# NVlabs/InstantSplat

Measured on AMD Instinct MI355X. Metric: train_iters_per_sec, higher is better.
Workload: dtype f32

## Files before the change

instantsplat_amd/csrc/adam.hip:

```cpp
#include <math.h>
#include "common.h"

namespace {

__global__ __launch_bounds__(256) void k_adam(int64_t n, int row, float* __restrict__ param, const float* __restrict__ grad,
                                               float* __restrict__ exp_avg, float* __restrict__ exp_avg_sq,
                                               const float* __restrict__ per_point_lr, const float* __restrict__ grad_sumsq,
                                               float step_size, float beta1, float beta2, float eps) {
  const bool update = grad_sumsq ? (*grad_sumsq > 0.f) : true;
  const int64_t stride = (int64_t)gridDim.x * blockDim.x;
  for (int64_t i = (int64_t)blockIdx.x * blockDim.x + threadIdx.x; i < n; i += stride) {
    float m = exp_avg[i];
    if (!update && m == 0.f) continue;
    float v = exp_avg_sq[i];
    if (update) {
      const float g = grad[i];
      m = m * beta1 + g * (1.f - beta1);
      v = v * beta2 + g * g * (1.f - beta2);
      exp_avg[i] = m;
      exp_avg_sq[i] = v;
    }
    const float denom = sqrtf(v) + eps;
    const float s = per_point_lr ? step_size * per_point_lr[i / row] : step_size;
    param[i] = param[i] - s * (m / denom);
  }
}

}

namespace {

constexpr int MT_MAX = 8;
constexpr int MT_CHUNK = 2048;

struct MultiAdamArgs {
  int n;
  int first_block[MT_MAX + 1];
  long long numel[MT_MAX];
  int row[MT_MAX];
  float* param[MT_MAX];
  const float* grad[MT_MAX];
  float* m[MT_MAX];
  float* v[MT_MAX];
  const float* pplr[MT_MAX];
  float step_size[MT_MAX];
  const float* gate;
  int gidx[MT_MAX];
  int sq_out[MT_MAX];
  int vec4[MT_MAX];
  uint32_t* live;
  uint32_t seq;
  const uint32_t* commit_count;
  unsigned long long commit_capacity;
  uint32_t* commit_poison;
};

__device__ __forceinline__ int mt_find(const MultiAdamArgs& a, int b) {
  int t = 0;
#pragma unroll
  for (int k = 1; k < MT_MAX; ++k) t += (k < a.n && b >= a.first_block[k]) ? 1 : 0;
  return t;
}

__global__ __launch_bounds__(256) void k_adam_sumsq(MultiAdamArgs a, float* __restrict__ sumsq) {
  __shared__ float s_red[4];
  const int t = mt_find(a, blockIdx.x);
  const long long lo = (long long)(blockIdx.x - a.first_block[t]) * MT_CHUNK;
  const long long hi = min(a.numel[t], lo + MT_CHUNK);
  const float* g = a.grad[t];
  float acc = 0.f;
  if (a.vec4[t]) {
    for (long long j = (lo >> 2) + threadIdx.x; j < (hi >> 2); j += 256) {
      const float4 x = reinterpret_cast<const float4*>(g)[j];
      acc += (x.x * x.x + x.y * x.y) + (x.z * x.z + x.w * x.w);
    }
  } else {
    for (long long i = lo + threadIdx.x; i < hi; i += 256) { const float x = g[i]; acc += x * x; }
  }
  acc = gs_wave_sum_row3(acc);
  if ((threadIdx.x & 63) == 63) s_red[threadIdx.x >> 6] = acc;
  __syncthreads();
  if (threadIdx.x == 0) {
    const float tot = (s_red[0] + s_red[1]) + (s_red[2] + s_red[3]);
    if (!(tot == 0.f)) atomicAdd(&sumsq[a.sq_out[t]], tot);
  }
}

__global__ __launch_bounds__(256) void k_adam_multi(MultiAdamArgs a, const float* __restrict__ sumsq, float beta1, float beta2,
                                                     float eps) {
  if (a.commit_count) {
    const bool over = (unsigned long long)*a.commit_count > a.commit_capacity;
    if (over || (a.commit_poison && *a.commit_poison)) {
      if (over && a.commit_poison && blockIdx.x == 0 && threadIdx.x == 0) *a.commit_poison = 1u;
      return;
    }
  }
  const int t = mt_find(a, blockIdx.x);
  const long long lo = (long long)(blockIdx.x - a.first_block[t]) * MT_CHUNK;
  const long long hi = min(a.numel[t], lo + MT_CHUNK);
  bool update;
  if (a.gidx[t] == -2) {
    __shared__ int s_any, s_nan;
    if (threadIdx.x == 0) { s_any = 0; s_nan = 0; }
    __syncthreads();
    bool nz = false, nan = false;
    for (long long i = lo + threadIdx.x; i < hi; i += 256) { const float x = a.grad[t][i]; nz = nz || x * x > 0.f; nan = nan || x != x; }
    if (nz) s_any = 1;
    if (nan) s_nan = 1;
    __syncthreads();
    update = s_any != 0 && s_nan == 0;
  } else {
    update = (a.gidx[t] >= 0 ? a.gate[a.gidx[t]] : sumsq[t]) > 0.f;
  }
  if (a.live) {
    const bool first = blockIdx.x == (unsigned)a.first_block[t] && threadIdx.x == 0;
    if (update) {
      if (first) { a.live[2 * t] = 0u; a.live[2 * t + 1] = 0u; }
    } else {
      const uint32_t scanned = a.live[2 * t], nonzero = a.live[2 * t + 1];
      if (scanned != 0u && scanned != a.seq && nonzero == 0u) return;
      if (first) a.live[2 * t] = a.seq;
    }
  }
  bool met_nonzero = false;
  float* __restrict__ p = a.param[t];
  const float* __restrict__ g = a.grad[t];
  float* __restrict__ mm = a.m[t];
  float* __restrict__ vv = a.v[t];
  const float* __restrict__ pplr = a.pplr[t];
  const int row = a.row[t];
  const float step_size = a.step_size[t];
  auto one = [&](float& pv, float gi, float& m, float& v, long long i) {
    if (update) {
      m = m * beta1 + gi * (1.f - beta1);
      v = v * beta2 + gi * gi * (1.f - beta2);
    }
    const float denom = sqrtf(v) + eps;
    const float s = pplr ? step_size * pplr[i / row] : step_size;
    pv = pv - s * (m / denom);
  };
  if (a.vec4[t]) {
    const long long vlo = lo >> 2, vhi = hi >> 2;
    for (long long j = vlo + threadIdx.x; j < vhi; j += 256) {
      float4 m4 = reinterpret_cast<const float4*>(mm)[j];
      if (!update && m4.x == 0.f && m4.y == 0.f && m4.z == 0.f && m4.w == 0.f) continue;
      met_nonzero = true;
      float4 v4 = reinterpret_cast<const float4*>(vv)[j];
      float4 p4 = reinterpret_cast<const float4*>(p)[j];
      float4 g4 = make_float4(0.f, 0.f, 0.f, 0.f);
      if (update) g4 = reinterpret_cast<const float4*>(g)[j];
      one(p4.x, g4.x, m4.x, v4.x, 4 * j); one(p4.y, g4.y, m4.y, v4.y, 4 * j + 1);
      one(p4.z, g4.z, m4.z, v4.z, 4 * j + 2); one(p4.w, g4.w, m4.w, v4.w, 4 * j + 3);
      if (update) { reinterpret_cast<float4*>(mm)[j] = m4; reinterpret_cast<float4*>(vv)[j] = v4; }
      reinterpret_cast<float4*>(p)[j] = p4;
    }
    if (a.live && !update && met_nonzero) a.live[2 * t + 1] = 1u;
    return;
  }
  for (long long i = lo + threadIdx.x; i < hi; i += 256) {
    float m = mm[i];
    if (!update && m == 0.f) continue;
    met_nonzero = true;
    float v = vv[i], pv = p[i];
    const float gi = update ? g[i] : 0.f;
    one(pv, gi, m, v, i);
    if (update) { mm[i] = m; vv[i] = v; }
    p[i] = pv;
  }
  if (a.live && !update && met_nonzero) a.live[2 * t + 1] = 1u;
}

}

extern "C" int mi355gs_adam_multi_step(void* stream_, int ntensors, const int64_t* numel, const int32_t* row, float* const* params,
                                       const float* const* grads, float* const* exp_avg, float* const* exp_avg_sq,
                                       const float* const* per_point_lr, const float* lr, float beta1, float beta2, float eps,
                                       const int32_t* step, float* scratch, const float* gate, const int32_t* gate_index,
                                       uint32_t* live, uint32_t seq) {
  GS_RANGE();
  hipStream_t stream = (hipStream_t)stream_;
  const int debug = 0;
  if (ntensors < 0 || ntensors > MT_MAX || (gate && !gate_index)) return MI355GS_EINVAL;
  if (ntensors == 0) return MI355GS_OK;
  if (!numel || !row || !params || !grads || !exp_avg || !exp_avg_sq || !per_point_lr || !lr || !step) return MI355GS_EINVAL;
  MultiAdamArgs a;
  a.n = ntensors; a.gate = gate;
  int blocks = 0;
  bool any_ungated = false;
  bool need_sumsq = false;
  for (int t = 0; t < MT_MAX; ++t) {
    a.first_block[t] = blocks;
    if (t < ntensors) {
      if (numel[t] < 0 || row[t] <= 0 || step[t] <= 0 || (numel[t] > 0 && (!params[t] || !grads[t] || !exp_avg[t] || !exp_avg_sq[t])))
        return MI355GS_EINVAL;
      if (gate && gate_index[t] >= MT_MAX) return MI355GS_EINVAL;
      a.numel[t] = numel[t]; a.row[t] = row[t]; a.gidx[t] = (gate && gate_index[t] >= 0) ? gate_index[t] : -1; a.sq_out[t] = t;
      if (a.gidx[t] < 0) any_ungated = true;
      a.param[t] = params[t]; a.grad[t] = grads[t]; a.m[t] = exp_avg[t]; a.v[t] = exp_avg_sq[t]; a.pplr[t] = per_point_lr[t];
      const double bc1 = 1.0 - pow((double)beta1, (double)step[t]), bc2 = 1.0 - pow((double)beta2, (double)step[t]);
      a.step_size[t] = (float)((double)lr[t] * (sqrt(bc2) / bc1));
      a.vec4[t] = (numel[t] % 4 == 0 && (((uintptr_t)params[t] | (uintptr_t)grads[t] | (uintptr_t)exp_avg[t] | (uintptr_t)exp_avg_sq[t]) & 15) == 0) ? 1 : 0;
      blocks += (int)((numel[t] + MT_CHUNK - 1) / MT_CHUNK);
    } else {
      a.numel[t] = 0; a.row[t] = 1; a.param[t] = nullptr; a.grad[t] = nullptr; a.m[t] = nullptr; a.v[t] = nullptr; a.pplr[t] = nullptr;
      a.step_size[t] = 0.f; a.vec4[t] = 0; a.gidx[t] = -1; a.sq_out[t] = t;
    }
  }
  a.first_block[MT_MAX] = blocks;
  a.live = nullptr; a.seq = 0; a.commit_count = nullptr; a.commit_capacity = 0; a.commit_poison = nullptr;
  if (blocks == 0) return MI355GS_OK;
  if (!gate && g_fused.gate == scratch) {
    a.live = g_fused.adam_live; a.seq = g_fused.adam_seq;
    a.commit_count = g_fused.commit_count; a.commit_capacity = g_fused.commit_capacity; a.commit_poison = g_fused.commit_poison;
  } else if (live && seq != 0u) {
    a.live = live; a.seq = seq;
  }
  if (gate && any_ungated) {
    for (int t = 0; t < ntensors; ++t) {
      if (a.gidx[t] >= 0) continue;
      if (a.numel[t] <= MT_CHUNK) a.gidx[t] = -2; else need_sumsq = true;
    }
  } else if (any_ungated) {
    need_sumsq = true;
  }
  if (need_sumsq && !scratch) return MI355GS_EINVAL;
  if (gate) {
    if (need_sumsq) {
      MultiAdamArgs s = a;
      int k = 0, sblocks = 0;
      for (int t = 0; t < ntensors; ++t) {
        if (a.gidx[t] != -1) continue;
        s.first_block[k] = sblocks; s.numel[k] = a.numel[t]; s.grad[k] = a.grad[t]; s.vec4[k] = a.vec4[t]; s.sq_out[k] = t;
        sblocks += (int)((a.numel[t] + MT_CHUNK - 1) / MT_CHUNK);
        ++k;
      }
      for (int j = k; j <= MT_MAX; ++j) s.first_block[j] = sblocks;
      s.n = k;
      if (hipMemsetAsync(scratch, 0, MT_MAX * sizeof(float), stream) != hipSuccess) return MI355GS_ELAUNCH;
      if (sblocks > 0) {
        GS_KRANGE("adam_sumsq");
        hipLaunchKernelGGL(k_adam_sumsq, dim3(sblocks), dim3(256), 0, stream, s, scratch);
        GS_CHECK_LAUNCH("adam_sumsq");
      }
    }
  } else if (g_fused.gate == scratch) {
    a.gate = scratch;
    for (int t = 0; t < ntensors; ++t) a.gidx[t] = t;
  } else {
    if (hipMemsetAsync(scratch, 0, MT_MAX * sizeof(float), stream) != hipSuccess) return MI355GS_ELAUNCH;
    GS_KRANGE("adam_sumsq");
    hipLaunchKernelGGL(k_adam_sumsq, dim3(blocks), dim3(256), 0, stream, a, scratch);
    GS_CHECK_LAUNCH("adam_sumsq");
  }
  GS_KRANGE("adam_multi");
  hipLaunchKernelGGL(k_adam_multi, dim3(blocks), dim3(256), 0, stream, a, (const float*)scratch, beta1, beta2, eps);
  GS_CHECK_LAUNCH("adam_multi");
  return MI355GS_OK;
}

extern "C" int mi355gs_adam_step(void* stream_, int64_t n, int row, float* param, const float* grad, float* exp_avg,
                                 float* exp_avg_sq, const float* per_point_lr, const float* grad_sumsq, float lr, float beta1,
                                 float beta2, float eps, int step) {
  GS_RANGE();
  hipStream_t stream = (hipStream_t)stream_;
  const int debug = 0;
  if (n < 0 || row <= 0 || step <= 0 || (n > 0 && (!param || !grad || !exp_avg || !exp_avg_sq))) return MI355GS_EINVAL;
  if (n == 0) return MI355GS_OK;
  const double bc1 = 1.0 - pow((double)beta1, (double)step), bc2 = 1.0 - pow((double)beta2, (double)step);
  const float step_size = (float)((double)lr * (sqrt(bc2) / bc1));
  int64_t blocks = (n + 255) / 256;
  if (blocks > 2048 * 4) blocks = 2048 * 4;
  GS_KRANGE("adam");
  hipLaunchKernelGGL(k_adam, dim3((unsigned)blocks), dim3(256), 0, stream, n, row, param, grad, exp_avg, exp_avg_sq, per_point_lr,
                     grad_sumsq, step_size, beta1, beta2, eps);
  GS_CHECK_LAUNCH("adam");
  return MI355GS_OK;
}
```

instantsplat_amd/csrc/preprocess.hip:

```cpp
#include "pose_math.h"

namespace {

constexpr float SH_C0 = 0.28209479177387814f;
constexpr float SH_C1 = 0.4886025119029199f;
constexpr float SH_C2_0 = 1.0925484305920792f, SH_C2_1 = -1.0925484305920792f, SH_C2_2 = 0.31539156525252005f,
                SH_C2_3 = -1.0925484305920792f, SH_C2_4 = 0.5462742152960396f;
constexpr float SH_C3_0 = -0.5900435899266435f, SH_C3_1 = 2.890611442640554f, SH_C3_2 = -0.4570457994644658f,
                SH_C3_3 = 0.3731763325901154f, SH_C3_4 = -0.4570457994644658f, SH_C3_5 = 1.445305721320277f,
                SH_C3_6 = -0.5900435899266435f;

struct Cov2D {
  float a, b, c;
};

struct Ewa {
  float tx, ty, tz, xmul, ymul;
  float M[6];
};

__device__ __forceinline__ Ewa ewa_setup(float3 pv, const float* view, const CamParams& cp) {
  Ewa e;
  const float limx = 1.3f * cp.tanfovx, limy = 1.3f * cp.tanfovy;
  const float txtz = pv.x / pv.z, tytz = pv.y / pv.z;
  e.tx = fminf(limx, fmaxf(-limx, txtz)) * pv.z;
  e.ty = fminf(limy, fmaxf(-limy, tytz)) * pv.z;
  e.tz = pv.z;
  e.xmul = (txtz < -limx || txtz > limx) ? 0.f : 1.f;
  e.ymul = (tytz < -limy || tytz > limy) ? 0.f : 1.f;
  const float j00 = cp.focal_x / e.tz, j02 = -(cp.focal_x * e.tx) / (e.tz * e.tz);
  const float j11 = cp.focal_y / e.tz, j12 = -(cp.focal_y * e.ty) / (e.tz * e.tz);
  e.M[0] = j00 * view[0] + j02 * view[2];
  e.M[1] = j00 * view[4] + j02 * view[6];
  e.M[2] = j00 * view[8] + j02 * view[10];
  e.M[3] = j11 * view[1] + j12 * view[2];
  e.M[4] = j11 * view[5] + j12 * view[6];
  e.M[5] = j11 * view[9] + j12 * view[10];
  return e;
}

__device__ __forceinline__ Cov2D ewa_cov2d(const Ewa& e, const float* cov) {
  const float* M = e.M;
  float MS[6];
  MS[0] = M[0] * cov[0] + M[1] * cov[1] + M[2] * cov[2];
  MS[1] = M[0] * cov[1] + M[1] * cov[3] + M[2] * cov[4];
  MS[2] = M[0] * cov[2] + M[1] * cov[4] + M[2] * cov[5];
  MS[3] = M[3] * cov[0] + M[4] * cov[1] + M[5] * cov[2];
  MS[4] = M[3] * cov[1] + M[4] * cov[3] + M[5] * cov[4];
  MS[5] = M[3] * cov[2] + M[4] * cov[4] + M[5] * cov[5];
  Cov2D c;
  c.a = MS[0] * M[0] + MS[1] * M[1] + MS[2] * M[2] + 0.3f;
  c.b = MS[0] * M[3] + MS[1] * M[4] + MS[2] * M[5];
  c.c = MS[3] * M[3] + MS[4] * M[4] + MS[5] * M[5] + 0.3f;
  return c;
}

__device__ __forceinline__ void quat_to_R(float r, float x, float y, float z, float* R) {
  R[0] = 1.f - 2.f * (y * y + z * z); R[1] = 2.f * (x * y - r * z); R[2] = 2.f * (x * z + r * y);
  R[3] = 2.f * (x * y + r * z); R[4] = 1.f - 2.f * (x * x + z * z); R[5] = 2.f * (y * z - r * x);
  R[6] = 2.f * (x * z - r * y); R[7] = 2.f * (y * z + r * x); R[8] = 1.f - 2.f * (x * x + y * y);
}

template <int NB>
__device__ __forceinline__ void sh_basis(float x, float y, float z, float* b) {
  b[0] = SH_C0;
  if (NB > 1) { b[1] = -SH_C1 * y; b[2] = SH_C1 * z; b[3] = -SH_C1 * x; }
  if (NB > 4) {
    const float xx = x * x, yy = y * y, zz = z * z, xy = x * y, yz = y * z, xz = x * z;
    b[4] = SH_C2_0 * xy; b[5] = SH_C2_1 * yz; b[6] = SH_C2_2 * (2.f * zz - xx - yy);
    b[7] = SH_C2_3 * xz; b[8] = SH_C2_4 * (xx - yy);
    if (NB > 9) {
      b[9] = SH_C3_0 * y * (3.f * xx - yy); b[10] = SH_C3_1 * xy * z;
      b[11] = SH_C3_2 * y * (4.f * zz - xx - yy); b[12] = SH_C3_3 * z * (2.f * zz - 3.f * xx - 3.f * yy);
      b[13] = SH_C3_4 * x * (4.f * zz - xx - yy); b[14] = SH_C3_5 * z * (xx - yy);
      b[15] = SH_C3_6 * x * (xx - 3.f * yy);
    }
  }
}

template <int NB>
__device__ __forceinline__ float3 sh_eval(const float* sh , float x, float y, float z) {
  float b[NB];
  sh_basis<NB>(x, y, z, b);
  float3 acc = make_float3(0.f, 0.f, 0.f);
#pragma unroll
  for (int k = 0; k < NB; ++k) {
    acc.x += b[k] * sh[3 * k]; acc.y += b[k] * sh[3 * k + 1]; acc.z += b[k] * sh[3 * k + 2];
  }
  return acc;
}

template <bool POSED, int D>
__global__ __launch_bounds__(256) void k_preprocess_fwd(
    int P, int M, const float* __restrict__ means3D, const float* __restrict__ shs, const float* __restrict__ shs_rest,
    const float* __restrict__ colors_precomp, const float* __restrict__ opacities, const float* __restrict__ scales,
    const float* __restrict__ rotations, const float* __restrict__ cov3D_precomp, CamParams cp,
    int32_t* __restrict__ radii, GsRec* __restrict__ recs, float* __restrict__ cov3Ds, uint2* __restrict__ rects,
    uint8_t* __restrict__ clamped, float* __restrict__ depths, uint8_t* __restrict__ visible, GsPosed posed, GsPrologue pro) {
  const int i = blockIdx.x * blockDim.x + threadIdx.x;
  {
    const size_t gid = (size_t)i, stride = (size_t)gridDim.x * blockDim.x;
    if (pro.grad_records) {
      const float4 z = make_float4(0.f, 0.f, 0.f, 0.f);
      for (size_t k = gid; k < pro.n_vec; k += stride) pro.grad_records[k] = z;
    }
    if (pro.tile_counters)
      for (size_t k = gid; k < (size_t)pro.n_counters; k += stride) pro.tile_counters[k] = 0u;
    if (pro.g_poses && gid < (size_t)pro.n_pose) pro.g_poses[gid] = 0.f;
    if (pro.pose_scratch && gid < 32) pro.pose_scratch[gid] = 0.f;
    if (pro.adam_scratch && gid < 8) pro.adam_scratch[gid] = 0.f;
  }
  if (i >= P) return;
  radii[i] = 0;
  if (visible) visible[i] = 0;
  rects[i] = make_uint2(0u, 0u);
  const float* view = cp.view;
  const float* proj = cp.proj;
  PoseMat pm;
  if (POSED) pm = load_pose(posed.pose);
  float3 m = make_float3(means3D[3 * (size_t)i], means3D[3 * (size_t)i + 1], means3D[3 * (size_t)i + 2]);
  if (POSED) m = pose_mean(pm, m.x, m.y, m.z);
  const float3 pv = gs_tp43(view, m);
  if (pv.z <= 0.2f) return;
  const float4 ph = gs_tp44(proj, m);
  const float pw = 1.0f / (ph.w + 0.0000001f);
  const float ndcx = ph.x * pw, ndcy = ph.y * pw;

  float cov[6];
  if (cov3D_precomp) {
#pragma unroll
    for (int k = 0; k < 6; ++k) cov[k] = cov3D_precomp[6 * (size_t)i + k];
  } else {
    float4 q = *reinterpret_cast<const float4*>(rotations + 4 * (size_t)i);
    float sc[3] = {scales[3 * (size_t)i], scales[3 * (size_t)i + 1], scales[3 * (size_t)i + 2]};
    if (POSED) {
      q = pose_rot(pm, q);
#pragma unroll
      for (int k = 0; k < 3; ++k) sc[k] = pose_scale(sc[k]);
    }
    float R[9];
    quat_to_R(q.x, q.y, q.z, q.w, R);
    const float s0 = cp.scale_modifier * sc[0], s1 = cp.scale_modifier * sc[1], s2 = cp.scale_modifier * sc[2];
    float L[9];
#pragma unroll
    for (int r = 0; r < 3; ++r) { L[3 * r] = R[3 * r] * s0; L[3 * r + 1] = R[3 * r + 1] * s1; L[3 * r + 2] = R[3 * r + 2] * s2; }
    cov[0] = L[0] * L[0] + L[1] * L[1] + L[2] * L[2];
    cov[1] = L[0] * L[3] + L[1] * L[4] + L[2] * L[5];
    cov[2] = L[0] * L[6] + L[1] * L[7] + L[2] * L[8];
    cov[3] = L[3] * L[3] + L[4] * L[4] + L[5] * L[5];
    cov[4] = L[3] * L[6] + L[4] * L[7] + L[5] * L[8];
    cov[5] = L[6] * L[6] + L[7] * L[7] + L[8] * L[8];
  }
#pragma unroll
  for (int k = 0; k < 6; ++k) cov3Ds[6 * (size_t)i + k] = cov[k];

  const Ewa e = ewa_setup(pv, view, cp);
  const Cov2D c2 = ewa_cov2d(e, cov);
  const float det = c2.a * c2.c - c2.b * c2.b;
  if (det == 0.0f) return;
  const float det_inv = 1.f / det;
  const float ca = c2.c * det_inv, cb = -c2.b * det_inv, cc = c2.a * det_inv;
  const float mid = 0.5f * (c2.a + c2.c);
  const float sq = sqrtf(fmaxf(0.1f, mid * mid - det));
  const float radius = ceilf(3.f * sqrtf(fmaxf(mid + sq, mid - sq)));
  const float px = ((ndcx + 1.0f) * cp.W - 1.0f) * 0.5f, py = ((ndcy + 1.0f) * cp.H - 1.0f) * 0.5f;
  const int rminx = min(cp.gx, max(0, (int)((px - radius) / GS_TILE)));
  const int rminy = min(cp.gy, max(0, (int)((py - radius) / GS_TILE)));
  const int rmaxx = min(cp.gx, max(0, (int)((px + radius + GS_TILE - 1) / GS_TILE)));
  const int rmaxy = min(cp.gy, max(0, (int)((py + radius + GS_TILE - 1) / GS_TILE)));
  if ((rmaxx - rminx) * (rmaxy - rminy) == 0) return;

  float3 rgb;
  uint8_t clamp_bits = 0;
  if (colors_precomp) {
    rgb = make_float3(colors_precomp[3 * (size_t)i], colors_precomp[3 * (size_t)i + 1], colors_precomp[3 * (size_t)i + 2]);
  } else {
    float dx = m.x - cp.campos[0], dy = m.y - cp.campos[1], dz = m.z - cp.campos[2];
    const float inv = 1.0f / sqrtf(dx * dx + dy * dy + dz * dz);
    dx *= inv; dy *= inv; dz *= inv;
    float3 v;
    constexpr int NBF = (D + 1) * (D + 1);
    if (shs_rest == nullptr) {
      v = sh_eval<NBF>(shs + (size_t)i * M * 3, dx, dy, dz);
    } else {
      float shl[NBF * 3];
      shl[0] = shs[3 * (size_t)i]; shl[1] = shs[3 * (size_t)i + 1]; shl[2] = shs[3 * (size_t)i + 2];
      const float* rest = shs_rest + (size_t)i * (M - 1) * 3;
#pragma unroll
      for (int k = 3; k < NBF * 3; ++k) shl[k] = rest[k - 3];
      v = sh_eval<NBF>(shl, dx, dy, dz);
    }
    v.x += 0.5f; v.y += 0.5f; v.z += 0.5f;
    clamp_bits = (uint8_t)((v.x < 0.f ? 1 : 0) | (v.y < 0.f ? 2 : 0) | (v.z < 0.f ? 4 : 0));
    rgb = make_float3(fmaxf(v.x, 0.f), fmaxf(v.y, 0.f), fmaxf(v.z, 0.f));
  }

  const float opac = POSED ? pose_opacity(opacities[i]) : opacities[i];
  float hx, hy;
  const float tau = __logf(255.0f * opac);
  const float cdet = ca * cc - cb * cb;
  if (!(tau > 0.f)) { hx = hy = -1e30f; }
  else if (!(cdet > 0.f) || ca * cc > 1000.f * cdet) { hx = hy = 1e30f; }
  else {
    const float s = 2.f * tau / cdet;
    hx = sqrtf(s * cc) * 1.01f + 0.5f;
    hy = sqrtf(s * ca) * 1.01f + 0.5f;
  }

  radii[i] = (int)radius;
  if (visible) visible[i] = 1;
  clamped[i] = clamp_bits;
  int bminx = rminx, bminy = rminy, bmaxx = rmaxx, bmaxy = rmaxy;
  if (hx < 1e29f) {
    if (hx < 0.f) { bmaxx = bminx; bmaxy = bminy; }
    else {
      bminx = max(bminx, (int)floorf((px - hx) * (1.0f / GS_TILE)));
      bminy = max(bminy, (int)floorf((py - hy) * (1.0f / GS_TILE)));
      bmaxx = min(bmaxx, (int)floorf((px + hx) * (1.0f / GS_TILE)) + 1);
      bmaxy = min(bmaxy, (int)floorf((py + hy) * (1.0f / GS_TILE)) + 1);
      if (bmaxx <= bminx || bmaxy <= bminy) { bmaxx = bminx; bmaxy = bminy; }
    }
  }
  rects[i] = make_uint2((uint32_t)bminx | ((uint32_t)bminy << 16), (uint32_t)bmaxx | ((uint32_t)bmaxy << 16));
  GsRec rec;
  rec.q0 = make_float4(px, py, hx, hy);
  rec.q1 = make_float4(-0.5f * GS_LOG2E * ca, -0.5f * GS_LOG2E * cc, -GS_LOG2E * cb, opac);
  rec.q2 = make_float4(rgb.x, rgb.y, rgb.z, pv.z);
  recs[i] = rec;
  depths[i] = pv.z;
}

template <int NB>
__device__ __forceinline__ void sh_backward(const float* sh, float* gsh, float x, float y, float z, float3 gr, float* gd) {
  float b[NB];
  sh_basis<NB>(x, y, z, b);
#pragma unroll
  for (int k = 0; k < NB; ++k) { gsh[3 * k] = b[k] * gr.x; gsh[3 * k + 1] = b[k] * gr.y; gsh[3 * k + 2] = b[k] * gr.z; }
  float w[NB];
#pragma unroll
  for (int k = 0; k < NB; ++k) w[k] = sh[3 * k] * gr.x + sh[3 * k + 1] * gr.y + sh[3 * k + 2] * gr.z;
  float gx = 0.f, gy = 0.f, gz = 0.f;
  if (NB > 1) { gy += -SH_C1 * w[1]; gz += SH_C1 * w[2]; gx += -SH_C1 * w[3]; }
  if (NB > 4) {
    const float xx = x * x, yy = y * y, zz = z * z;
    gx += SH_C2_0 * y * w[4]; gy += SH_C2_0 * x * w[4];
    gy += SH_C2_1 * z * w[5]; gz += SH_C2_1 * y * w[5];
    gx += SH_C2_2 * -2.f * x * w[6]; gy += SH_C2_2 * -2.f * y * w[6]; gz += SH_C2_2 * 4.f * z * w[6];
    gx += SH_C2_3 * z * w[7]; gz += SH_C2_3 * x * w[7];
    gx += SH_C2_4 * 2.f * x * w[8]; gy += SH_C2_4 * -2.f * y * w[8];
    if (NB > 9) {
      gx += SH_C3_0 * 6.f * x * y * w[9]; gy += SH_C3_0 * (3.f * xx - 3.f * yy) * w[9];
      gx += SH_C3_1 * y * z * w[10]; gy += SH_C3_1 * x * z * w[10]; gz += SH_C3_1 * x * y * w[10];
      gx += SH_C3_2 * -2.f * x * y * w[11]; gy += SH_C3_2 * (4.f * zz - xx - 3.f * yy) * w[11]; gz += SH_C3_2 * 8.f * y * z * w[11];
      gx += SH_C3_3 * -6.f * x * z * w[12]; gy += SH_C3_3 * -6.f * y * z * w[12]; gz += SH_C3_3 * (6.f * zz - 3.f * xx - 3.f * yy) * w[12];
      gx += SH_C3_4 * (4.f * zz - 3.f * xx - yy) * w[13]; gy += SH_C3_4 * -2.f * x * y * w[13]; gz += SH_C3_4 * 8.f * x * z * w[13];
      gx += SH_C3_5 * 2.f * x * z * w[14]; gy += SH_C3_5 * -2.f * y * z * w[14]; gz += SH_C3_5 * (xx - yy) * w[14];
      gx += SH_C3_6 * (3.f * xx - 3.f * yy) * w[15]; gy += SH_C3_6 * -6.f * x * y * w[15];
    }
  }
  gd[0] = gx; gd[1] = gy; gd[2] = gz;
}

template <bool POSED, int D, bool POSE_ONLY = false>
__global__ __launch_bounds__(256) void k_preprocess_bwd(
    int P, int M, const float* __restrict__ means3D, const float* __restrict__ shs, const float* __restrict__ shs_rest,
    const float* __restrict__ scales, const float* __restrict__ rotations, int use_shs, int use_cov_precomp, CamParams cp, const int32_t* __restrict__ radii,
    const GsRec* __restrict__ recs, const float* __restrict__ cov3Ds, const uint8_t* __restrict__ clamped, const GsGrad* __restrict__ grads,
    float* __restrict__ dL_dmeans3D, float* __restrict__ dL_dmeans2D, float* __restrict__ dL_dshs, float* __restrict__ dL_dshs_rest,
    float* __restrict__ dL_dcolors, float* __restrict__ dL_dopac, float* __restrict__ dL_dscales,
    float* __restrict__ dL_drots, float* __restrict__ dL_dcov3D, float* __restrict__ sh_gate, float* __restrict__ sh_rest_gate,
    GsPosed posed, float* __restrict__ gate, int gi_xyz, int gi_rot, int gi_scaling, int gi_opacity) {
  __shared__ float s_red[POSED ? 4 : 1][16];
  const int i_raw = blockIdx.x * blockDim.x + threadIdx.x;
  if (!POSED && i_raw >= P) return;
  const bool live = i_raw < P;
  const int i = live ? i_raw : 0;
  const bool vis = live && radii[i] > 0;
  PoseMat pm;
  if (POSED) pm = load_pose(posed.pose);
  GsGrad g;
  g.g0 = make_float4(0, 0, 0, 0); g.g1 = g.g0; g.g2 = g.g0;
  if (vis) {
    const GsGrad mo = grads[i];
    const float4 pre = recs[i].q1;
    const float4 con = make_float4(pre.x * (-2.0f / GS_LOG2E), pre.z * (-1.0f / GS_LOG2E), pre.y * (-2.0f / GS_LOG2E), pre.w);
    const float m1 = mo.g0.x, m2 = mo.g0.y, m3 = mo.g0.z, m4 = mo.g0.w, m5 = mo.g1.x, m0 = mo.g1.y;
    g.g0.x = -(con.x * m1 + con.y * m2) * (0.5f * cp.W);
    g.g0.y = -(con.z * m2 + con.y * m1) * (0.5f * cp.H);
    g.g0.z = -0.5f * m3;
    g.g0.w = -m4;
    g.g1.x = -0.5f * m5;
    g.g1.y = con.w != 0.f ? m0 / con.w : 0.f;
    g.g1.z = mo.g1.z; g.g1.w = mo.g1.w; g.g2.x = mo.g2.x;
  }
  float gm[3] = {0.f, 0.f, 0.f};
  float gcov[6] = {0.f, 0.f, 0.f, 0.f, 0.f, 0.f};
  float gs[3] = {0.f, 0.f, 0.f}, gq[4] = {0.f, 0.f, 0.f, 0.f};
  const float3 gcol = make_float3(g.g1.z, g.g1.w, g.g2.x);
  constexpr int nb = (D + 1) * (D + 1);
  const bool split = shs_rest != nullptr;
  float gsh_local[nb * 3];

  if (vis) {
    const float* view = cp.view;
    const float* proj = cp.proj;
    float3 m = make_float3(means3D[3 * (size_t)i], means3D[3 * (size_t)i + 1], means3D[3 * (size_t)i + 2]);
    if (POSED) m = pose_mean(pm, m.x, m.y, m.z);
    float cov[6];
#pragma unroll
    for (int k = 0; k < 6; ++k) cov[k] = cov3Ds[6 * (size_t)i + k];
    {
      const float3 pv = gs_tp43(view, m);
      const Ewa e = ewa_setup(pv, view, cp);
      const Cov2D c2 = ewa_cov2d(e, cov);
      const float a = c2.a, b = c2.b, c = c2.c;
      const float det = a * c - b * b;
      const float Dv = 1.f / (det * det + 0.0000001f);
      const float gA = g.g0.z, gB = g.g0.w, gC = g.g1.x;
      const float ga = Dv * (-c * c * gA + b * c * gB + (det - a * c) * gC);
      const float gc = Dv * ((det - a * c) * gA + a * b * gB - a * a * gC);
      const float gb = Dv * (2.f * b * c * gA - (det + 2.f * b * b) * gB + 2.f * a * b * gC);
      const float* Mx = e.M;
      float GM[6];
#pragma unroll
      for (int k = 0; k < 3; ++k) { GM[k] = ga * Mx[k] + 0.5f * gb * Mx[3 + k]; GM[3 + k] = 0.5f * gb * Mx[k] + gc * Mx[3 + k]; }
      gcov[0] = Mx[0] * GM[0] + Mx[3] * GM[3];
      gcov[1] = 2.f * (Mx[0] * GM[1] + Mx[3] * GM[4]);
      gcov[2] = 2.f * (Mx[0] * GM[2] + Mx[3] * GM[5]);
      gcov[3] = Mx[1] * GM[1] + Mx[4] * GM[4];
      gcov[4] = 2.f * (Mx[1] * GM[2] + Mx[4] * GM[5]);
      gcov[5] = Mx[2] * GM[2] + Mx[5] * GM[5];
      float gM[6];
      gM[0] = 2.f * (GM[0] * cov[0] + GM[1] * cov[1] + GM[2] * cov[2]);
      gM[1] = 2.f * (GM[0] * cov[1] + GM[1] * cov[3] + GM[2] * cov[4]);
      gM[2] = 2.f * (GM[0] * cov[2] + GM[1] * cov[4] + GM[2] * cov[5]);
      gM[3] = 2.f * (GM[3] * cov[0] + GM[4] * cov[1] + GM[5] * cov[2]);
      gM[4] = 2.f * (GM[3] * cov[1] + GM[4] * cov[3] + GM[5] * cov[4]);
      gM[5] = 2.f * (GM[3] * cov[2] + GM[4] * cov[4] + GM[5] * cov[5]);
      const float gJ00 = gM[0] * view[0] + gM[1] * view[4] + gM[2] * view[8];
      const float gJ02 = gM[0] * view[2] + gM[1] * view[6] + gM[2] * view[10];
      const float gJ11 = gM[3] * view[1] + gM[4] * view[5] + gM[5] * view[9];
      const float gJ12 = gM[3] * view[2] + gM[4] * view[6] + gM[5] * view[10];
      const float tz2 = 1.f / (e.tz * e.tz), tz3 = tz2 / e.tz;
      const float gtx = e.xmul * -cp.focal_x * tz2 * gJ02;
      const float gty = e.ymul * -cp.focal_y * tz2 * gJ12;
      const float gtz = -cp.focal_x * tz2 * gJ00 - cp.focal_y * tz2 * gJ11 + 2.f * cp.focal_x * e.tx * tz3 * gJ02 +
                        2.f * cp.focal_y * e.ty * tz3 * gJ12;
      gm[0] = view[0] * gtx + view[1] * gty + view[2] * gtz;
      gm[1] = view[4] * gtx + view[5] * gty + view[6] * gtz;
      gm[2] = view[8] * gtx + view[9] * gty + view[10] * gtz;
    }
    {
      const float4 ph = gs_tp44(proj, m);
      const float mw = 1.0f / (ph.w + 0.0000001f);
      const float mul1 = ph.x * mw * mw, mul2 = ph.y * mw * mw;
      const float g2x = g.g0.x, g2y = g.g0.y;
      gm[0] += (proj[0] * mw - proj[3] * mul1) * g2x + (proj[1] * mw - proj[3] * mul2) * g2y;
      gm[1] += (proj[4] * mw - proj[7] * mul1) * g2x + (proj[5] * mw - proj[7] * mul2) * g2y;
      gm[2] += (proj[8] * mw - proj[11] * mul1) * g2x + (proj[9] * mw - proj[11] * mul2) * g2y;
    }
    if (use_shs) {
      float dx = m.x - cp.campos[0], dy = m.y - cp.campos[1], dz = m.z - cp.campos[2];
      const float inv = 1.0f / sqrtf(dx * dx + dy * dy + dz * dz);
      dx *= inv; dy *= inv; dz *= inv;
      const uint8_t cl = clamped[i];
      const float3 gr = make_float3((cl & 1) ? 0.f : gcol.x, (cl & 2) ? 0.f : gcol.y, (cl & 4) ? 0.f : gcol.z);
      float shl[nb * 3];
      if (split) {
        shl[0] = shs[3 * (size_t)i]; shl[1] = shs[3 * (size_t)i + 1]; shl[2] = shs[3 * (size_t)i + 2];
        const float* rest = shs_rest + (size_t)i * (M - 1) * 3;
#pragma unroll
        for (int k = 3; k < nb * 3; ++k) shl[k] = rest[k - 3];
      } else {
        const float* src = shs + (size_t)i * M * 3;
#pragma unroll
        for (int k = 0; k < nb * 3; ++k) shl[k] = src[k];
      }
      float gd[3];
      sh_backward<nb>(shl, gsh_local, dx, dy, dz, gr, gd);
      const float dot = dx * gd[0] + dy * gd[1] + dz * gd[2];
      gm[0] += (gd[0] - dx * dot) * inv; gm[1] += (gd[1] - dy * dot) * inv; gm[2] += (gd[2] - dz * dot) * inv;
    }
    if (!use_cov_precomp) {
      float4 q = *reinterpret_cast<const float4*>(rotations + 4 * (size_t)i);
      float sc[3] = {scales[3 * (size_t)i], scales[3 * (size_t)i + 1], scales[3 * (size_t)i + 2]};
      if (POSED) {
        q = pose_rot(pm, q);
#pragma unroll
        for (int k = 0; k < 3; ++k) sc[k] = pose_scale(sc[k]);
      }
      float R[9];
      quat_to_R(q.x, q.y, q.z, q.w, R);
      const float mod = cp.scale_modifier;
      const float s[3] = {mod * sc[0], mod * sc[1], mod * sc[2]};
      float L[9];
#pragma unroll
      for (int r = 0; r < 3; ++r) { L[3 * r] = R[3 * r] * s[0]; L[3 * r + 1] = R[3 * r + 1] * s[1]; L[3 * r + 2] = R[3 * r + 2] * s[2]; }
      const float Gs[9] = {gcov[0], 0.5f * gcov[1], 0.5f * gcov[2], 0.5f * gcov[1], gcov[3], 0.5f * gcov[4],
                           0.5f * gcov[2], 0.5f * gcov[4], gcov[5]};
      float gL[9];
#pragma unroll
      for (int r = 0; r < 3; ++r)
#pragma unroll
        for (int k = 0; k < 3; ++k) gL[3 * r + k] = 2.f * (Gs[3 * r] * L[k] + Gs[3 * r + 1] * L[3 + k] + Gs[3 * r + 2] * L[6 + k]);
      float Rp[9];
#pragma unroll
      for (int k = 0; k < 3; ++k) {
        gs[k] = cp.scale_grad_factor * (R[k] * gL[k] + R[3 + k] * gL[3 + k] + R[6 + k] * gL[6 + k]);
#pragma unroll
        for (int r = 0; r < 3; ++r) Rp[3 * r + k] = gL[3 * r + k] * s[k];
      }
      const float r_ = q.x, x = q.y, y = q.z, z = q.w;
      gq[0] = 2.f * (z * (Rp[3] - Rp[1]) + y * (Rp[2] - Rp[6]) + x * (Rp[7] - Rp[5]));
      gq[1] = 2.f * (y * (Rp[1] + Rp[3]) + z * (Rp[2] + Rp[6]) + r_ * (Rp[7] - Rp[5])) - 4.f * x * (Rp[4] + Rp[8]);
      gq[2] = 2.f * (x * (Rp[1] + Rp[3]) + r_ * (Rp[2] - Rp[6]) + z * (Rp[5] + Rp[7])) - 4.f * y * (Rp[0] + Rp[8]);
      gq[3] = 2.f * (r_ * (Rp[3] - Rp[1]) + x * (Rp[2] + Rp[6]) + y * (Rp[5] + Rp[7])) - 4.f * z * (Rp[0] + Rp[4]);
    }
  }

  if (live && !POSE_ONLY) {
    if (!POSED) {
      dL_dmeans3D[3 * (size_t)i] = gm[0]; dL_dmeans3D[3 * (size_t)i + 1] = gm[1]; dL_dmeans3D[3 * (size_t)i + 2] = gm[2];
      dL_dopac[i] = g.g1.y;
      if (dL_dscales) { dL_dscales[3 * (size_t)i] = gs[0]; dL_dscales[3 * (size_t)i + 1] = gs[1]; dL_dscales[3 * (size_t)i + 2] = gs[2]; }
      if (dL_drots) *reinterpret_cast<float4*>(dL_drots + 4 * (size_t)i) = make_float4(gq[0], gq[1], gq[2], gq[3]);
    }
    dL_dmeans2D[3 * (size_t)i] = g.g0.x; dL_dmeans2D[3 * (size_t)i + 1] = g.g0.y; dL_dmeans2D[3 * (size_t)i + 2] = 0.f;
    if (dL_dcolors) { dL_dcolors[3 * (size_t)i] = gcol.x; dL_dcolors[3 * (size_t)i + 1] = gcol.y; dL_dcolors[3 * (size_t)i + 2] = gcol.z; }
    if (dL_dshs) {
      const bool have = vis && use_shs;
      bool nz_dc = false, nz_rest = false;
      if (!split) {
        float* gdst = dL_dshs + (size_t)i * M * 3;
#pragma unroll
        for (int k = 0; k < nb * 3; ++k) { const float v = have ? gsh_local[k] : 0.f; gdst[k] = v; nz_dc = nz_dc || v != 0.f; }
        for (int k = nb * 3; k < M * 3; ++k) gdst[k] = 0.f;
      } else {
        float* gdc = dL_dshs + 3 * (size_t)i;
#pragma unroll
        for (int c = 0; c < 3; ++c) { const float v = have ? gsh_local[c] : 0.f; gdc[c] = v; nz_dc = nz_dc || v != 0.f; }
        if (dL_dshs_rest) {
          float* grest = dL_dshs_rest + (size_t)i * (M - 1) * 3;
#pragma unroll
          for (int k = 3; k < nb * 3; ++k) { const float v = have ? gsh_local[k] : 0.f; grest[k - 3] = v; nz_rest = nz_rest || v != 0.f; }
          for (int k = nb * 3; k < M * 3; ++k) grest[k - 3] = 0.f;
        }
      }
      if (sh_gate && nz_dc) *sh_gate = 1.0f;
      if (sh_rest_gate && nz_rest) *sh_rest_gate = 1.0f;
    }
    if (dL_dcov3D) {
      const bool on = vis && use_cov_precomp;
#pragma unroll
      for (int k = 0; k < 6; ++k) dL_dcov3D[6 * (size_t)i + k] = on ? gcov[k] : 0.f;
    }
  }
  if (POSED) {
    float a[16];
#pragma unroll
    for (int k = 0; k < 16; ++k) a[k] = 0.f;
    bool nz_xyz = false, nz_rot = false, nz_sc = false, nz_op = false;
    if (live) {
      float act[3];
#pragma unroll
      for (int k = 0; k < 3; ++k) act[k] = pose_scale(scales[3 * (size_t)i + k]);
      const float o = vis ? recs[i].q1.w : 0.5f;
      const PoseGradOut r = pose_backward_one(pm, means3D[3 * (size_t)i], means3D[3 * (size_t)i + 1], means3D[3 * (size_t)i + 2],
                                              *reinterpret_cast<const float4*>(rotations + 4 * (size_t)i), act, o, gm[0], gm[1], gm[2],
                                              make_float4(gq[0], gq[1], gq[2], gq[3]), gs, g.g1.y, a);
      if (!POSE_ONLY) {
#pragma unroll
        for (int k = 0; k < 3; ++k) {
          dL_dmeans3D[3 * (size_t)i + k] = r.d_xyz[k];
          dL_dscales[3 * (size_t)i + k] = r.d_scaling[k];
          nz_xyz = nz_xyz || r.d_xyz[k] != 0.f;
          nz_sc = nz_sc || r.d_scaling[k] != 0.f;
        }
        *reinterpret_cast<float4*>(dL_drots + 4 * (size_t)i) = r.d_rot;
        nz_rot = nz_rot || r.d_rot.x != 0.f || r.d_rot.y != 0.f || r.d_rot.z != 0.f || r.d_rot.w != 0.f;
        dL_dopac[i] = r.d_opacity_logit;
        nz_op = nz_op || r.d_opacity_logit != 0.f;
      }
    }
    pose_accumulate(a, posed.acc, posed.partial, s_red);
    if (!POSE_ONLY && gate) {
      if (gi_xyz >= 0 && nz_xyz) gate[gi_xyz] = 1.0f;
      if (gi_rot >= 0 && nz_rot) gate[gi_rot] = 1.0f;
      if (gi_scaling >= 0 && nz_sc) gate[gi_scaling] = 1.0f;
      if (gi_opacity >= 0 && nz_op) gate[gi_opacity] = 1.0f;
    }
  }
}

__global__ __launch_bounds__(256) void k_mark_visible(int P, const float* __restrict__ means3D, const float* __restrict__ view,
                                                      uint8_t* __restrict__ present) {
  const int i = blockIdx.x * blockDim.x + threadIdx.x;
  if (i >= P) return;
  const float3 m = make_float3(means3D[3 * (size_t)i], means3D[3 * (size_t)i + 1], means3D[3 * (size_t)i + 2]);
  present[i] = gs_tp43(view, m).z > 0.2f ? 1 : 0;
}

}

int gs_launch_preprocess_fwd(hipStream_t stream, int P, int D, int M, const float* means3D, const float* shs, const float* shs_rest,
                             const float* colors_precomp, const float* opacities, const float* scales,
                             const float* rotations, const float* cov3D_precomp, const CamParams& cp, int32_t* radii,
                             GsRec* recs, float* cov3Ds, uint2* rects, uint8_t* clamped, float* depths, uint8_t* visible,
                             const GsPrologue& pro) {
  if (P <= 0) return 0;
  const bool posed = g_fused.posed.pose != nullptr;
  const GsPosed pa = posed ? g_fused.posed : GsPosed();
#define GS_FWD(POSED, DEG)                                                                                                              \
  hipLaunchKernelGGL((k_preprocess_fwd<POSED, DEG>), dim3((P + 255) / 256), dim3(256), 0, stream, P, M, means3D, shs, shs_rest,         \
                     colors_precomp, opacities, scales, rotations, cov3D_precomp, cp, radii, recs, cov3Ds, rects, clamped, depths, visible, pa, pro)
  const int deg = shs ? D : 0;
  if (posed) { if (deg == 0) GS_FWD(true, 0); else if (deg == 1) GS_FWD(true, 1); else if (deg == 2) GS_FWD(true, 2); else GS_FWD(true, 3); }
  else { if (deg == 0) GS_FWD(false, 0); else if (deg == 1) GS_FWD(false, 1); else if (deg == 2) GS_FWD(false, 2); else GS_FWD(false, 3); }
#undef GS_FWD
  return 0;
}

// ... 32 lines not shown
```

Before: 3543.

## Persistent-grid Adam with 2x unroll; hoist loads and recompute cov3D in backward

The multi-tensor Adam kernel now runs a grid-stride loop over chunks with a grid capped at a resident-block count, and the update path is unrolled twice to keep more memory loads in flight. Preprocess stops writing cov3Ds when covariance is computed from rotation and scale, and the backward pass recomputes it from R and S instead of reading it back. Both preprocess and backward now issue all per-point loads up front, which costs more registers and loads data for culled points. Recomputing covariance adds arithmetic and relies on no other reader needing the cov3Ds buffer.

```diff
diff --git a/instantsplat_amd/csrc/adam.hip b/instantsplat_amd/csrc/adam.hip
--- a/instantsplat_amd/csrc/adam.hip
+++ b/instantsplat_amd/csrc/adam.hip
@@ -32,6 +32,7 @@
 
 constexpr int MT_MAX = 8;
 constexpr int MT_CHUNK = 2048;
+constexpr int MT_RESIDENT_BLOCKS = 256 * 7;
 
 struct MultiAdamArgs {
   int n;
@@ -86,21 +87,15 @@
   }
 }
 
-__global__ __launch_bounds__(256) void k_adam_multi(MultiAdamArgs a, const float* __restrict__ sumsq, float beta1, float beta2,
-                                                     float eps) {
-  if (a.commit_count) {
-    const bool over = (unsigned long long)*a.commit_count > a.commit_capacity;
-    if (over || (a.commit_poison && *a.commit_poison)) {
-      if (over && a.commit_poison && blockIdx.x == 0 && threadIdx.x == 0) *a.commit_poison = 1u;
-      return;
-    }
-  }
-  const int t = mt_find(a, blockIdx.x);
-  const long long lo = (long long)(blockIdx.x - a.first_block[t]) * MT_CHUNK;
+__device__ __forceinline__ void adam_chunk(const MultiAdamArgs& a, const float* __restrict__ sumsq, int b, float beta1, float beta2,
+                                           float eps) {
+  const int t = mt_find(a, b);
+  const long long lo = (long long)(b - a.first_block[t]) * MT_CHUNK;
   const long long hi = min(a.numel[t], lo + MT_CHUNK);
   bool update;
   if (a.gidx[t] == -2) {
     __shared__ int s_any, s_nan;
+    __syncthreads();
     if (threadIdx.x == 0) { s_any = 0; s_nan = 0; }
     __syncthreads();
     bool nz = false, nan = false;
@@ -113,7 +108,7 @@
     update = (a.gidx[t] >= 0 ? a.gate[a.gidx[t]] : sumsq[t]) > 0.f;
   }
   if (a.live) {
-    const bool first = blockIdx.x == (unsigned)a.first_block[t] && threadIdx.x == 0;
+    const bool first = b == a.first_block[t] && threadIdx.x == 0;
     if (update) {
       if (first) { a.live[2 * t] = 0u; a.live[2 * t + 1] = 0u; }
     } else {
@@ -141,6 +136,29 @@
   };
   if (a.vec4[t]) {
     const long long vlo = lo >> 2, vhi = hi >> 2;
+    float4* __restrict__ p4s = reinterpret_cast<float4*>(p);
+    float4* __restrict__ m4s = reinterpret_cast<float4*>(mm);
+    float4* __restrict__ v4s = reinterpret_cast<float4*>(vv);
+    const float4* __restrict__ g4s = reinterpret_cast<const float4*>(g);
+    if (update) {
+      for (long long j = vlo + threadIdx.x; j < vhi; j += 512) {
+        const long long j1 = j + 256;
+        const bool two = j1 < vhi;
+        float4 m0 = m4s[j], v0 = v4s[j], p0 = p4s[j];
+        const float4 g0 = g4s[j];
+        float4 m1 = m0, v1 = v0, p1 = p0, g1 = g0;
+        if (two) { m1 = m4s[j1]; v1 = v4s[j1]; p1 = p4s[j1]; g1 = g4s[j1]; }
+        one(p0.x, g0.x, m0.x, v0.x, 4 * j); one(p0.y, g0.y, m0.y, v0.y, 4 * j + 1);
+        one(p0.z, g0.z, m0.z, v0.z, 4 * j + 2); one(p0.w, g0.w, m0.w, v0.w, 4 * j + 3);
+        m4s[j] = m0; v4s[j] = v0; p4s[j] = p0;
+        if (two) {
+          one(p1.x, g1.x, m1.x, v1.x, 4 * j1); one(p1.y, g1.y, m1.y, v1.y, 4 * j1 + 1);
+          one(p1.z, g1.z, m1.z, v1.z, 4 * j1 + 2); one(p1.w, g1.w, m1.w, v1.w, 4 * j1 + 3);
+          m4s[j1] = m1; v4s[j1] = v1; p4s[j1] = p1;
+        }
+      }
+      return;
+    }
     for (long long j = vlo + threadIdx.x; j < vhi; j += 256) {
       float4 m4 = reinterpret_cast<const float4*>(mm)[j];
       if (!update && m4.x == 0.f && m4.y == 0.f && m4.z == 0.f && m4.w == 0.f) continue;
@@ -168,6 +186,18 @@
     p[i] = pv;
   }
   if (a.live && !update && met_nonzero) a.live[2 * t + 1] = 1u;
+}
+
+__global__ __launch_bounds__(256) void k_adam_multi(MultiAdamArgs a, const float* __restrict__ sumsq, float beta1, float beta2,
+                                                     float eps) {
+  if (a.commit_count) {
+    const bool over = (unsigned long long)*a.commit_count > a.commit_capacity;
+    if (over || (a.commit_poison && *a.commit_poison)) {
+      if (over && a.commit_poison && blockIdx.x == 0 && threadIdx.x == 0) *a.commit_poison = 1u;
+      return;
+    }
+  }
+  for (int b = blockIdx.x; b < a.first_block[MT_MAX]; b += gridDim.x) adam_chunk(a, sumsq, b, beta1, beta2, eps);
 }
 
 }
@@ -253,7 +283,8 @@
     GS_CHECK_LAUNCH("adam_sumsq");
   }
   GS_KRANGE("adam_multi");
-  hipLaunchKernelGGL(k_adam_multi, dim3(blocks), dim3(256), 0, stream, a, (const float*)scratch, beta1, beta2, eps);
+  hipLaunchKernelGGL(k_adam_multi, dim3(blocks < MT_RESIDENT_BLOCKS ? blocks : MT_RESIDENT_BLOCKS), dim3(256), 0, stream, a,
+                     (const float*)scratch, beta1, beta2, eps);
   GS_CHECK_LAUNCH("adam_multi");
   return MI355GS_OK;
 }
diff --git a/instantsplat_amd/csrc/preprocess.hip b/instantsplat_amd/csrc/preprocess.hip
--- a/instantsplat_amd/csrc/preprocess.hip
+++ b/instantsplat_amd/csrc/preprocess.hip
@@ -61,6 +61,17 @@
   R[6] = 2.f * (x * z - r * y); R[7] = 2.f * (y * z + r * x); R[8] = 1.f - 2.f * (x * x + y * y);
 }
 
+__device__ __forceinline__ void cov3d_from_RS(const float* R, float s0, float s1, float s2, float* L, float* cov) {
+#pragma unroll
+  for (int r = 0; r < 3; ++r) { L[3 * r] = R[3 * r] * s0; L[3 * r + 1] = R[3 * r + 1] * s1; L[3 * r + 2] = R[3 * r + 2] * s2; }
+  cov[0] = L[0] * L[0] + L[1] * L[1] + L[2] * L[2];
+  cov[1] = L[0] * L[3] + L[1] * L[4] + L[2] * L[5];
+  cov[2] = L[0] * L[6] + L[1] * L[7] + L[2] * L[8];
+  cov[3] = L[3] * L[3] + L[4] * L[4] + L[5] * L[5];
+  cov[4] = L[3] * L[6] + L[4] * L[7] + L[5] * L[8];
+  cov[5] = L[6] * L[6] + L[7] * L[7] + L[8] * L[8];
+}
+
 template <int NB>
 __device__ __forceinline__ void sh_basis(float x, float y, float z, float* b) {
   b[0] = SH_C0;
@@ -111,53 +122,69 @@
     if (pro.adam_scratch && gid < 8) pro.adam_scratch[gid] = 0.f;
   }
   if (i >= P) return;
-  radii[i] = 0;
-  if (visible) visible[i] = 0;
-  rects[i] = make_uint2(0u, 0u);
+  constexpr int NBF = (D + 1) * (D + 1);
+  float3 m = make_float3(means3D[3 * (size_t)i], means3D[3 * (size_t)i + 1], means3D[3 * (size_t)i + 2]);
+  float cov[6];
+  float4 q = make_float4(0.f, 0.f, 0.f, 0.f);
+  float sc[3] = {0.f, 0.f, 0.f};
+  if (cov3D_precomp) {
+#pragma unroll
+    for (int k = 0; k < 6; ++k) cov[k] = cov3D_precomp[6 * (size_t)i + k];
+  } else {
+    q = *reinterpret_cast<const float4*>(rotations + 4 * (size_t)i);
+#pragma unroll
+    for (int k = 0; k < 3; ++k) sc[k] = scales[3 * (size_t)i + k];
+  }
+  const float opac_in = opacities[i];
+  float3 rgb = make_float3(0.f, 0.f, 0.f);
+  float shl[NBF * 3];
+  if (colors_precomp) {
+    rgb = make_float3(colors_precomp[3 * (size_t)i], colors_precomp[3 * (size_t)i + 1], colors_precomp[3 * (size_t)i + 2]);
+  } else if (shs_rest == nullptr) {
+    const float* src = shs + (size_t)i * M * 3;
+#pragma unroll
+    for (int k = 0; k < NBF * 3; ++k) shl[k] = src[k];
+  } else {
+    shl[0] = shs[3 * (size_t)i]; shl[1] = shs[3 * (size_t)i + 1]; shl[2] = shs[3 * (size_t)i + 2];
+    const float* rest = shs_rest + (size_t)i * (M - 1) * 3;
+#pragma unroll
+    for (int k = 3; k < NBF * 3; ++k) shl[k] = rest[k - 3];
+  }
+  auto cull = [&]() {
+    radii[i] = 0;
+    if (visible) visible[i] = 0;
+    rects[i] = make_uint2(0u, 0u);
+  };
+
   const float* view = cp.view;
   const float* proj = cp.proj;
   PoseMat pm;
   if (POSED) pm = load_pose(posed.pose);
-  float3 m = make_float3(means3D[3 * (size_t)i], means3D[3 * (size_t)i + 1], means3D[3 * (size_t)i + 2]);
   if (POSED) m = pose_mean(pm, m.x, m.y, m.z);
   const float3 pv = gs_tp43(view, m);
-  if (pv.z <= 0.2f) return;
+  if (pv.z <= 0.2f) { cull(); return; }
   const float4 ph = gs_tp44(proj, m);
   const float pw = 1.0f / (ph.w + 0.0000001f);
   const float ndcx = ph.x * pw, ndcy = ph.y * pw;
 
-  float cov[6];
-  if (cov3D_precomp) {
-#pragma unroll
-    for (int k = 0; k < 6; ++k) cov[k] = cov3D_precomp[6 * (size_t)i + k];
-  } else {
-    float4 q = *reinterpret_cast<const float4*>(rotations + 4 * (size_t)i);
-    float sc[3] = {scales[3 * (size_t)i], scales[3 * (size_t)i + 1], scales[3 * (size_t)i + 2]};
+  if (!cov3D_precomp) {
     if (POSED) {
       q = pose_rot(pm, q);
 #pragma unroll
       for (int k = 0; k < 3; ++k) sc[k] = pose_scale(sc[k]);
     }
-    float R[9];
+    float R[9], L[9];
     quat_to_R(q.x, q.y, q.z, q.w, R);
-    const float s0 = cp.scale_modifier * sc[0], s1 = cp.scale_modifier * sc[1], s2 = cp.scale_modifier * sc[2];
-    float L[9];
-#pragma unroll
-    for (int r = 0; r < 3; ++r) { L[3 * r] = R[3 * r] * s0; L[3 * r + 1] = R[3 * r + 1] * s1; L[3 * r + 2] = R[3 * r + 2] * s2; }
-    cov[0] = L[0] * L[0] + L[1] * L[1] + L[2] * L[2];
-    cov[1] = L[0] * L[3] + L[1] * L[4] + L[2] * L[5];
-    cov[2] = L[0] * L[6] + L[1] * L[7] + L[2] * L[8];
-    cov[3] = L[3] * L[3] + L[4] * L[4] + L[5] * L[5];
-    cov[4] = L[3] * L[6] + L[4] * L[7] + L[5] * L[8];
-    cov[5] = L[6] * L[6] + L[7] * L[7] + L[8] * L[8];
-  }
-#pragma unroll
-  for (int k = 0; k < 6; ++k) cov3Ds[6 * (size_t)i + k] = cov[k];
+    cov3d_from_RS(R, cp.scale_modifier * sc[0], cp.scale_modifier * sc[1], cp.scale_modifier * sc[2], L, cov);
+  } else {
+#pragma unroll
+    for (int k = 0; k < 6; ++k) cov3Ds[6 * (size_t)i + k] = cov[k];
+  }
 
   const Ewa e = ewa_setup(pv, view, cp);
   const Cov2D c2 = ewa_cov2d(e, cov);
   const float det = c2.a * c2.c - c2.b * c2.b;
-  if (det == 0.0f) return;
+  if (det == 0.0f) { cull(); return; }
   const float det_inv = 1.f / det;
   const float ca = c2.c * det_inv, cb = -c2.b * det_inv, cc = c2.a * det_inv;
   const float mid = 0.5f * (c2.a + c2.c);
@@ -168,34 +195,20 @@
   const int rminy = min(cp.gy, max(0, (int)((py - radius) / GS_TILE)));
   const int rmaxx = min(cp.gx, max(0, (int)((px + radius + GS_TILE - 1) / GS_TILE)));
   const int rmaxy = min(cp.gy, max(0, (int)((py + radius + GS_TILE - 1) / GS_TILE)));
-  if ((rmaxx - rminx) * (rmaxy - rminy) == 0) return;
-
-  float3 rgb;
+  if ((rmaxx - rminx) * (rmaxy - rminy) == 0) { cull(); return; }
+
   uint8_t clamp_bits = 0;
-  if (colors_precomp) {
-    rgb = make_float3(colors_precomp[3 * (size_t)i], colors_precomp[3 * (size_t)i + 1], colors_precomp[3 * (size_t)i + 2]);
-  } else {
+  if (!colors_precomp) {
     float dx = m.x - cp.campos[0], dy = m.y - cp.campos[1], dz = m.z - cp.campos[2];
     const float inv = 1.0f / sqrtf(dx * dx + dy * dy + dz * dz);
     dx *= inv; dy *= inv; dz *= inv;
-    float3 v;
-    constexpr int NBF = (D + 1) * (D + 1);
-    if (shs_rest == nullptr) {
-      v = sh_eval<NBF>(shs + (size_t)i * M * 3, dx, dy, dz);
-    } else {
-      float shl[NBF * 3];
-      shl[0] = shs[3 * (size_t)i]; shl[1] = shs[3 * (size_t)i + 1]; shl[2] = shs[3 * (size_t)i + 2];
-      const float* rest = shs_rest + (size_t)i * (M - 1) * 3;
-#pragma unroll
-      for (int k = 3; k < NBF * 3; ++k) shl[k] = rest[k - 3];
-      v = sh_eval<NBF>(shl, dx, dy, dz);
-    }
+    float3 v = sh_eval<NBF>(shl, dx, dy, dz);
     v.x += 0.5f; v.y += 0.5f; v.z += 0.5f;
     clamp_bits = (uint8_t)((v.x < 0.f ? 1 : 0) | (v.y < 0.f ? 2 : 0) | (v.z < 0.f ? 4 : 0));
     rgb = make_float3(fmaxf(v.x, 0.f), fmaxf(v.y, 0.f), fmaxf(v.z, 0.f));
   }
 
-  const float opac = POSED ? pose_opacity(opacities[i]) : opacities[i];
+  const float opac = POSED ? pose_opacity(opac_in) : opac_in;
   float hx, hy;
   const float tau = __logf(255.0f * opac);
   const float cdet = ca * cc - cb * cb;
@@ -275,14 +288,45 @@
   if (!POSED && i_raw >= P) return;
   const bool live = i_raw < P;
   const int i = live ? i_raw : 0;
-  const bool vis = live && radii[i] > 0;
+  constexpr int nb = (D + 1) * (D + 1);
+  const bool split = shs_rest != nullptr;
+  const int32_t radius = radii[i];
+  const float3 m_raw = make_float3(means3D[3 * (size_t)i], means3D[3 * (size_t)i + 1], means3D[3 * (size_t)i + 2]);
+  float4 q_raw = make_float4(0.f, 0.f, 0.f, 0.f);
+  float sc_raw[3] = {0.f, 0.f, 0.f};
+  float cov[6];
+  if (POSED || !use_cov_precomp) {
+    q_raw = *reinterpret_cast<const float4*>(rotations + 4 * (size_t)i);
+#pragma unroll
+    for (int k = 0; k < 3; ++k) sc_raw[k] = scales[3 * (size_t)i + k];
+  }
+  if (use_cov_precomp) {
+#pragma unroll
+    for (int k = 0; k < 6; ++k) cov[k] = cov3Ds[6 * (size_t)i + k];
+  }
+  const GsGrad mo = grads[i];
+  const float4 pre = recs[i].q1;
+  uint8_t cl = 0;
+  float shl[nb * 3];
+  if (use_shs) {
+    cl = clamped[i];
+    if (split) {
+      shl[0] = shs[3 * (size_t)i]; shl[1] = shs[3 * (size_t)i + 1]; shl[2] = shs[3 * (size_t)i + 2];
+      const float* rest = shs_rest + (size_t)i * (M - 1) * 3;
+#pragma unroll
+      for (int k = 3; k < nb * 3; ++k) shl[k] = rest[k - 3];
+    } else {
+      const float* src = shs + (size_t)i * M * 3;
+#pragma unroll
+      for (int k = 0; k < nb * 3; ++k) shl[k] = src[k];
+    }
+  }
+  const bool vis = live && radius > 0;
   PoseMat pm;
   if (POSED) pm = load_pose(posed.pose);
   GsGrad g;
   g.g0 = make_float4(0, 0, 0, 0); g.g1 = g.g0; g.g2 = g.g0;
   if (vis) {
-    const GsGrad mo = grads[i];
-    const float4 pre = recs[i].q1;
     const float4 con = make_float4(pre.x * (-2.0f / GS_LOG2E), pre.z * (-1.0f / GS_LOG2E), pre.y * (-2.0f / GS_LOG2E), pre.w);
     const float m1 = mo.g0.x, m2 = mo.g0.y, m3 = mo.g0.z, m4 = mo.g0.w, m5 = mo.g1.x, m0 = mo.g1.y;
     g.g0.x = -(con.x * m1 + con.y * m2) * (0.5f * cp.W);
@@ -297,18 +341,28 @@
   float gcov[6] = {0.f, 0.f, 0.f, 0.f, 0.f, 0.f};
   float gs[3] = {0.f, 0.f, 0.f}, gq[4] = {0.f, 0.f, 0.f, 0.f};
   const float3 gcol = make_float3(g.g1.z, g.g1.w, g.g2.x);
-  constexpr int nb = (D + 1) * (D + 1);
-  const bool split = shs_rest != nullptr;
   float gsh_local[nb * 3];
 
   if (vis) {
     const float* view = cp.view;
     const float* proj = cp.proj;
-    float3 m = make_float3(means3D[3 * (size_t)i], means3D[3 * (size_t)i + 1], means3D[3 * (size_t)i + 2]);
+    float3 m = m_raw;
     if (POSED) m = pose_mean(pm, m.x, m.y, m.z);
-    float cov[6];
-#pragma unroll
-    for (int k = 0; k < 6; ++k) cov[k] = cov3Ds[6 * (size_t)i + k];
+    float4 q = q_raw;
+    float s[3], R[9], L[9];
+    if (!use_cov_precomp) {
+      float sc[3] = {sc_raw[0], sc_raw[1], sc_raw[2]};
+      if (POSED) {
+        q = pose_rot(pm, q);
+#pragma unroll
+        for (int k = 0; k < 3; ++k) sc[k] = pose_scale(sc[k]);
+      }
+      quat_to_R(q.x, q.y, q.z, q.w, R);
+      const float mod = cp.scale_modifier;
+#pragma unroll
+      for (int k = 0; k < 3; ++k) s[k] = mod * sc[k];
+      cov3d_from_RS(R, s[0], s[1], s[2], L, cov);
+    }
     {
       const float3 pv = gs_tp43(view, m);
       const Ewa e = ewa_setup(pv, view, cp);
@@ -363,39 +417,13 @@
       float dx = m.x - cp.campos[0], dy = m.y - cp.campos[1], dz = m.z - cp.campos[2];
       const float inv = 1.0f / sqrtf(dx * dx + dy * dy + dz * dz);
       dx *= inv; dy *= inv; dz *= inv;
-      const uint8_t cl = clamped[i];
       const float3 gr = make_float3((cl & 1) ? 0.f : gcol.x, (cl & 2) ? 0.f : gcol.y, (cl & 4) ? 0.f : gcol.z);
-      float shl[nb * 3];
-      if (split) {
-        shl[0] = shs[3 * (size_t)i]; shl[1] = shs[3 * (size_t)i + 1]; shl[2] = shs[3 * (size_t)i + 2];
-        const float* rest = shs_rest + (size_t)i * (M - 1) * 3;
-#pragma unroll
-        for (int k = 3; k < nb * 3; ++k) shl[k] = rest[k - 3];
-      } else {
-        const float* src = shs + (size_t)i * M * 3;
-#pragma unroll
-        for (int k = 0; k < nb * 3; ++k) shl[k] = src[k];
-      }
       float gd[3];
       sh_backward<nb>(shl, gsh_local, dx, dy, dz, gr, gd);
       const float dot = dx * gd[0] + dy * gd[1] + dz * gd[2];
       gm[0] += (gd[0] - dx * dot) * inv; gm[1] += (gd[1] - dy * dot) * inv; gm[2] += (gd[2] - dz * dot) * inv;
     }
     if (!use_cov_precomp) {
-      float4 q = *reinterpret_cast<const float4*>(rotations + 4 * (size_t)i);
-      float sc[3] = {scales[3 * (size_t)i], scales[3 * (size_t)i + 1], scales[3 * (size_t)i + 2]};
-      if (POSED) {
-        q = pose_rot(pm, q);
-#pragma unroll
-        for (int k = 0; k < 3; ++k) sc[k] = pose_scale(sc[k]);
-      }
-      float R[9];
-      quat_to_R(q.x, q.y, q.z, q.w, R);
-      const float mod = cp.scale_modifier;
-      const float s[3] = {mod * sc[0], mod * sc[1], mod * sc[2]};
-      float L[9];
-#pragma unroll
-      for (int r = 0; r < 3; ++r) { L[3 * r] = R[3 * r] * s[0]; L[3 * r + 1] = R[3 * r + 1] * s[1]; L[3 * r + 2] = R[3 * r + 2] * s[2]; }
       const float Gs[9] = {gcov[0], 0.5f * gcov[1], 0.5f * gcov[2], 0.5f * gcov[1], gcov[3], 0.5f * gcov[4],
                            0.5f * gcov[2], 0.5f * gcov[4], gcov[5]};
       float gL[9];
@@ -463,10 +491,9 @@
     if (live) {
       float act[3];
 #pragma unroll
-      for (int k = 0; k < 3; ++k) act[k] = pose_scale(scales[3 * (size_t)i + k]);
-      const float o = vis ? recs[i].q1.w : 0.5f;
-      const PoseGradOut r = pose_backward_one(pm, means3D[3 * (size_t)i], means3D[3 * (size_t)i + 1], means3D[3 * (size_t)i + 2],
-                                              *reinterpret_cast<const float4*>(rotations + 4 * (size_t)i), act, o, gm[0], gm[1], gm[2],
+      for (int k = 0; k < 3; ++k) act[k] = pose_scale(sc_raw[k]);
+      const float o = vis ? pre.w : 0.5f;
+      const PoseGradOut r = pose_backward_one(pm, m_raw.x, m_raw.y, m_raw.z, q_raw, act, o, gm[0], gm[1], gm[2],
                                               make_float4(gq[0], gq[1], gq[2], gq[3]), gs, g.g1.y, a);
       if (!POSE_ONLY) {
 #pragma unroll
```

After: 3504, median of 3. Within noise of the previous version (-1.1%).
